# Polochon-street/bliss

Hardware: AMD Instinct MI355X
Metric: songs/sec bl_analyze (3-min 44.1kHz s16) + 10k x 10k distance-matrix sec (higher is better)
Workload: dtype f64; 1 GPU; configs[2] shard: 8192 synthetic 180-s 44.1 kHz s16 stereo songs/GPU resident (260.1 GB), 8192 total; step = analyze + all-gather + row-block distance; songs_per_gpu=8192, parallelism=shard1, fir_mode=2

## Files before the change

### bliss_amd/csrc/bl_stats_kernels.hip

```cpp
#include <hip/hip_runtime.h>
#include <math.h>

#include "bl_launch.h"
#include "bl_scan.h"
#include "bl_fir.h"


template <bool HIST>
__global__ __launch_bounds__(256) void k_pcm_scan(const int16_t *__restrict__ pcm,
                                                  const bl_dsong *__restrict__ songs,
                                                  bl_dstats *stats, unsigned *hist) {
  __shared__ unsigned lh[BL_HIST_BINS];
  if (__builtin_amdgcn_groupstaticsize() != sizeof lh) __builtin_trap();
  const int tid = threadIdx.x;
  const bl_dsong sg = songs[blockIdx.y];
  const int16_t *p = pcm + sg.pcm_off;
  for (int i = tid; i < BL_HIST_BINS; i += 256) lh[i] = 0;
  __syncthreads();
  unsigned lds_base = (unsigned)(size_t)(bl_lds_u32 *)lh;
  asm volatile("" : "+v"(lds_base));

  long long sum = 0;
  unsigned long long sq = 0;
  const unsigned nvec = (unsigned)sg.n >> 3;
  const uint4 *pv = reinterpret_cast<const uint4 *>(p);
  auto eat = [&](const uint4 q) {
    const unsigned w[4] = {q.x, q.y, q.z, q.w};
    int s32 = 0;
#pragma unroll
    for (int k = 0; k < 4; ++k) scan_word(w[k], s32, sq, lds_base, HIST);
    sum += s32;
  };
  const unsigned gstride = gridDim.x * 256u;
  unsigned v = blockIdx.x * 256u + tid;
  for (; v + gstride < nvec; v += 2 * gstride) {
    const uint4 q0 = pv[v], q1 = pv[v + gstride];
    eat(q0);
    eat(q1);
  }
  if (v < nvec) eat(pv[v]);
  if (blockIdx.x == 0 && tid < (sg.n & 7)) {
    const int sv = (int)p[8u * nvec + tid];
    sum += sv;
    sq += (unsigned)(sv * sv);
    const unsigned b = (unsigned)(sv + BL_HIST_BINS / 2);
    if (HIST && b < BL_HIST_BINS) atomicAdd(&lh[b], 1u);
  }
#pragma unroll
  for (int off = 32; off > 0; off >>= 1) {
    sum += __shfl_down(sum, off);
    sq += __shfl_down(sq, off);
  }
  bl_dstats *st = stats + blockIdx.y;
  if ((tid & 63) == 0) {
    atomicAdd(&st->sum, (unsigned long long)sum);
    atomicAdd(&st->sumsq, sq);
  }
  asm volatile("s_waitcnt lgkmcnt(0)" ::: "memory");
  __syncthreads();
  unsigned *gh = hist + (size_t)blockIdx.y * BL_HIST_BINS;
  for (int i = tid; i < BL_HIST_BINS; i += 256) {
    const unsigned c = lh[i];
    if (c) atomicAdd(&gh[i], c);
  }
}

__global__ __launch_bounds__(128) void k_trim(const int16_t *__restrict__ pcm, const bl_dsong *__restrict__ songs,
                                              bl_dstats *stats) {
  const bl_dsong sg = songs[blockIdx.x];
  const int16_t *p = pcm + sg.pcm_off;
  const uint4 *pv = reinterpret_cast<const uint4 *>(p);
  const int lane = threadIdx.x & 63, n = sg.n;
  const int nvec = n >> 3;
  const bool fwd = __builtin_amdgcn_readfirstlane(threadIdx.x >> 6) == 0;
  bl_dstats *st = stats + blockIdx.x;
  auto locate = [&](const uint4 q) -> int {
    const unsigned w[4] = {q.x, q.y, q.z, q.w};
    int at = fwd ? 8 : -1;
#pragma unroll
    for (int k = 0; k < 4; ++k) {
      if (fwd) {
        if (w[3 - k] >> 16) at = 2 * (3 - k) + 1;
        if (w[3 - k] & 0xFFFFu) at = 2 * (3 - k);
      } else {
        if (w[k] & 0xFFFFu) at = 2 * k;
        if (w[k] >> 16) at = 2 * k + 1;
      }
    }
    return at;
  };
  if (fwd) {
    unsigned first = 0xFFFFFFFFu;
    for (int v0 = 0; v0 < nvec; v0 += 128) {
      const int va = v0 + lane, vb = v0 + 64 + lane;
      const uint4 z = make_uint4(0, 0, 0, 0);
      const uint4 qa = va < nvec ? pv[va] : z, qb = vb < nvec ? pv[vb] : z;
      const unsigned long long ma = __ballot((qa.x | qa.y | qa.z | qa.w) != 0u);
      const unsigned long long mb = __ballot((qb.x | qb.y | qb.z | qb.w) != 0u);
      if (ma | mb) {
        const int src = ma ? __builtin_ctzll(ma) : __builtin_ctzll(mb);
        const unsigned mine = 8u * (unsigned)(ma ? va : vb) + (unsigned)locate(ma ? qa : qb);
        first = (unsigned)__shfl((int)mine, src);
        break;
      }
    }
    if (first == 0xFFFFFFFFu)
      for (int i = 8 * nvec; i < n; ++i)
        if (p[i] != 0) { first = (unsigned)i; break; }
    if (lane == 0) st->first = first;
  } else {
    int last = -1;
    for (int i = n - 1; i >= 8 * nvec; --i)
      if (p[i] != 0) { last = i; break; }
    if (last < 0)
      for (int v1 = nvec; v1 > 0; v1 -= 128) {
        const int va = v1 - 1 - lane, vb = v1 - 65 - lane;
        const uint4 z = make_uint4(0, 0, 0, 0);
        const uint4 qa = va >= 0 ? pv[va] : z, qb = vb >= 0 ? pv[vb] : z;
        const unsigned long long ma = __ballot((qa.x | qa.y | qa.z | qa.w) != 0u);
        const unsigned long long mb = __ballot((qb.x | qb.y | qb.z | qb.w) != 0u);
        if (ma | mb) {
          const int src = ma ? __builtin_ctzll(ma) : __builtin_ctzll(mb);
          const int mine = 8 * (ma ? va : vb) + locate(ma ? qa : qb);
          last = __shfl(mine, src);
          break;
        }
      }
    if (lane == 0) st->last = last;
  }
}

__global__ void k_stats_init(bl_dstats *stats, int n_songs) {
  const int i = blockIdx.x * blockDim.x + threadIdx.x;
  if (i >= n_songs) return;
  bl_dstats s;
  s.sum = 0; s.sumsq = 0; s.first = 0xFFFFFFFFu; s.last = -1;
  s.mean = 0; s.variance = 0; s.vprime = 0; s.rcp = 0; s.rcp_lo = 0; s.fsc = 0; s.kappa = 0; s.wrap_pass = 0; s.status = BL_OK;
  s.wrap_acc = 0;
  stats[i] = s;
}


__device__ __forceinline__ void prep_finish(bl_dstats &s, int n) {
  if (s.variance == 0) s.status = BL_UNEXPECTED;
  s.vprime = (double)s.variance / 32768.0;
  const double v2 = 2.0 * s.vprime;
  s.rcp = 1.0 / v2;
  s.rcp_lo = __builtin_fma(-s.rcp, v2, 1.0) / v2;
  s.fsc = bl_firi_scale(s.rcp, s.rcp_lo);
  s.kappa = bl_firi_power_scale(s.rcp, s.rcp_lo);
  (void)n;
}

__global__ void k_song_prep(const bl_dsong *__restrict__ songs, bl_dstats *stats, int n_songs,
                            bl_amd_song_result *res) {
  const int i = blockIdx.x * blockDim.x + threadIdx.x;
  if (i >= n_songs) return;
  bl_dstats s = stats[i];
  const bl_dsong sg = songs[i];
  const int n = sg.n;
  if (s.first == 0xFFFFFFFFu) {
    s.status = BL_UNEXPECTED;
    s.first = 0; s.last = n - 1;
  }
  const int wrapped = (int)(unsigned)(s.sum & 0xFFFFFFFFull);
  s.mean = wrapped / n;
  const long long m = s.mean;
  if (m > 13571 || m < -13571) {
    s.wrap_pass = 1;
  } else {
    const long long acc = (long long)s.sumsq - 2 * m * (long long)s.sum + (long long)n * m * m;
    s.variance = (int)(acc / n);
    prep_finish(s, n);
  }
  stats[i] = s;
  bl_amd_song_result *r = res + sg.out_idx;
  r->start = (int)s.first; r->end = s.last;
  r->mean = s.mean; r->variance = s.variance;
  r->n_frames = sg.n_frames; r->nb_frames = sg.nb_frames; r->n_windows = sg.n_windows;
  r->status = s.status;
}

__global__ __launch_bounds__(256) void k_variance_wrap(const int16_t *__restrict__ pcm,
                                                       const bl_dsong *__restrict__ songs,
                                                       bl_dstats *stats) {
  bl_dstats *st = stats + blockIdx.y;
  if (!st->wrap_pass) return;
  const bl_dsong sg = songs[blockIdx.y];
  const int16_t *p = pcm + sg.pcm_off;
  const int mean = st->mean;
  long long acc = 0;
  for (unsigned i = blockIdx.x * 256u + threadIdx.x; i < (unsigned)sg.n; i += gridDim.x * 256u) {
    const int v = (int)p[i] - mean;
    acc += (int)((unsigned)v * (unsigned)v);
  }
#pragma unroll
  for (int off = 32; off > 0; off >>= 1) acc += __shfl_down(acc, off);
  if ((threadIdx.x & 63) == 0)
    atomicAdd(reinterpret_cast<unsigned long long *>(&st->wrap_acc), (unsigned long long)acc);
}

__global__ void k_variance_wrap_finish(const bl_dsong *__restrict__ songs, bl_dstats *stats,
                                       int n_songs, bl_amd_song_result *res) {
  const int i = blockIdx.x * blockDim.x + threadIdx.x;
  if (i >= n_songs) return;
  bl_dstats s = stats[i];
  if (!s.wrap_pass) return;
  s.variance = (int)(s.wrap_acc / songs[i].n);
  prep_finish(s, songs[i].n);
  stats[i] = s;
  res[songs[i].out_idx].variance = s.variance;
  res[songs[i].out_idx].status = s.status;
}


#define BL_AMP_PASSES 301
#define BL_INT_LO ((32767 - 1000) - BL_HIST_LO)
#define BL_INT_HI ((32767 + 1000) - BL_HIST_LO)

__global__ __launch_bounds__(256) void k_amp_finish(const bl_dsong *__restrict__ songs,
                                                    const bl_dstats *__restrict__ stats,
                                                    const unsigned *__restrict__ hist,
                                                    bl_amd_song_result *res) {
  __shared__ float buf[2][BL_HIST_BINS + 8];
  const int tid = threadIdx.x;
  const int song = blockIdx.x;
  const bl_dstats st = stats[song];
  const int n = songs[song].n;
  const unsigned *gh = hist + (size_t)song * BL_HIST_BINS;
  const int start = (int)st.first, end = st.last;
  if (tid < 8) {
    const int c = tid < 3 ? tid : BL_HIST_BINS + tid;
    buf[0][c] = 0.f; buf[1][c] = 0.f;
  }
  for (int i = tid; i < BL_HIST_BINS; i += 256) {
    unsigned c = gh[i];
    if (i == BL_HIST_BINS / 2) c -= (unsigned)start + (unsigned)(n - 1 - end);
    buf[0][i + 3] = (float)min(c, 16777216u);
  }
  __syncthreads();
  int cur = 0;
  for (int g = 0; g < BL_AMP_PASSES; ++g) {
    const float *h = buf[cur] + 3;
    float *s = buf[cur ^ 1] + 3;
    const int reach = 3 * (BL_AMP_PASSES - 1 - g);
    const int lo = max(BL_INT_LO - reach, 0), hi = min(BL_INT_HI + reach, BL_HIST_BINS - 1);
    for (int i = lo + tid; i <= hi; i += 256) {
      float acc = h[i - 3] + (3 * h[i - 2]);
      acc = acc + (6 * h[i - 1]);
      acc = acc + (7 * h[i]);
      acc = acc + (6 * h[i + 1]);
      acc = acc + (3 * h[i + 2]);
      acc = acc + h[i + 3];
      s[i] = (float)(1. / 27. * (double)acc);
    }
    __syncthreads();
    cur ^= 1;
  }
  float *s = buf[cur] + 3;
  float *v = buf[cur ^ 1] + 3;
  const float denom = (float)(start - end);
  for (int i = BL_INT_LO + tid; i <= BL_INT_HI; i += 256) {
    float t = s[i] / denom;
    t = (float)((double)t * 100.);
    v[i] = fabsf(t);
  }
  __syncthreads();
  if (tid == 0) {
    float integral = 0;
    for (int i = BL_INT_LO; i <= BL_INT_HI; ++i) integral += v[i];
    bl_amd_song_result *r = res + songs[song].out_idx;
    r->hist_integral = integral;
    r->v.amplitude = -0.2f * integral + 6.0f;
  }
}

__global__ void k_force(bl_amd_song_result *res, int n_songs) {
  const int i = blockIdx.x * blockDim.x + threadIdx.x;
  if (i >= n_songs) return;
  bl_amd_song_result *r = res + i;
  const float rating = (float)(fmax((double)r->v.tempo, 0.0) + (double)r->v.amplitude +
                               (double)r->v.frequency + fmax((double)r->v.attack, 0.0));
  r->force = rating;
  r->calm_or_loud = rating > 0 ? BL_LOUD : (rating < 0 ? BL_CALM : BL_UNKNOWN);
}


static int scan_grid_x(int max_n, int n_songs, int n_cu) {
  return grid_x_for(((long long)max_n / 8 + 255) / 256, n_songs, 8, n_cu);
}

void blk_stats_init(const blk_analyze_args &a) {
  hipLaunchKernelGGL(k_stats_init, dim3((a.n_songs + 63) / 64), dim3(64), 0, a.stream, a.stats, a.n_songs);
}

int blk_pcm_scan(const blk_analyze_args &a) {
  BL_HIP_CHECK(hipMemsetAsync(a.hist, 0, sizeof(unsigned) * BL_HIST_BINS * (size_t)a.n_songs, a.stream));
  Mark m(a.mark, a.mark_user, PK_SCAN, a.stream);
  hipLaunchKernelGGL(k_pcm_scan<true>, dim3(scan_grid_x(a.max_n, a.n_songs, a.n_cu), a.n_songs), dim3(256), 0,
                     a.stream, a.pcm, a.songs, a.stats, a.hist);
  return BL_OK;
}

void blk_song_prep(const blk_analyze_args &a) {
  const int n_songs = a.n_songs, tb64 = (n_songs + 63) / 64;
  hipStream_t stream = a.stream;
  hipLaunchKernelGGL(k_trim, dim3(n_songs), dim3(128), 0, stream, a.pcm, a.songs, a.stats);
  hipLaunchKernelGGL(k_song_prep, dim3(tb64), dim3(64), 0, stream, a.songs, a.stats, n_songs,
                     a.results);
  hipLaunchKernelGGL(k_variance_wrap, dim3(scan_grid_x(a.max_n, n_songs, a.n_cu), n_songs), dim3(256), 0, stream,
                     a.pcm, a.songs, a.stats);
  hipLaunchKernelGGL(k_variance_wrap_finish, dim3(tb64), dim3(64), 0, stream, a.songs, a.stats,
                     n_songs, a.results);
}

void blk_amp_finish(const blk_analyze_args &a, hipStream_t s) {
  Mark m(a.mark, a.mark_user, PK_AMP, s);
  hipLaunchKernelGGL(k_amp_finish, dim3(a.n_songs), dim3(256), 0, s, a.songs, a.stats, a.hist,
                     a.results);
}

void blk_force(const blk_analyze_args &a) {
  hipLaunchKernelGGL(k_force, dim3((a.n_songs + 63) / 64), dim3(64), 0, a.stream, a.results, a.n_songs);
}

int blk_scan_one(hipStream_t s, const int16_t *pcm, const bl_dsong *d_songs, bl_dstats *d_stats,
                 unsigned *d_hist, int n, int n_cu) {
  const int gx = scan_grid_x(n, 1, n_cu);
  BL_HIP_CHECK(hipMemsetAsync(d_hist, 0, sizeof(unsigned) * BL_HIST_BINS, s));
  hipLaunchKernelGGL(k_stats_init, dim3(1), dim3(64), 0, s, d_stats, 1);
  hipLaunchKernelGGL(k_pcm_scan<true>, dim3(gx, 1), dim3(256), 0, s, pcm, d_songs, d_stats, d_hist);
  hipLaunchKernelGGL(k_trim, dim3(1), dim3(128), 0, s, pcm, d_songs, d_stats);
  BL_HIP_CHECK(hipGetLastError());
  return BL_OK;
}

int blk_variance_wrap_one(hipStream_t s, const int16_t *pcm, const bl_dsong *d_songs,
                          bl_dstats *d_stats, int n, int n_cu) {
  const int gx = scan_grid_x(n, 1, n_cu);
  hipLaunchKernelGGL(k_variance_wrap, dim3(gx, 1), dim3(256), 0, s, pcm, d_songs, d_stats);
  BL_HIP_CHECK(hipGetLastError());
  return BL_OK;
}
```

Before: 25490 songs/s.

## Run amplitude histogram smoothing passes in registers within one wavefront using DPP

Rewrites k_amp_finish so one 64-lane wave holds the histogram bins needed by the integral in registers, 60 per lane. Each of the 301 smoothing passes exchanges halo values between neighbouring lanes with DPP row shifts instead of going through LDS with a barrier per pass. Counts are loaded as 16-byte vectors, and the serial integral sum is replaced by per-lane sums chained through readlane. Register pressure is high (two 60-float arrays plus temporaries). The DPP row_shl/row_shr controls (0x138/0x130) shift within 16-lane rows, not across the full wave, so halo values at row boundaries may be wrong.

```diff
diff --git a/bliss_amd/csrc/bl_stats_kernels.hip b/bliss_amd/csrc/bl_stats_kernels.hip
--- a/bliss_amd/csrc/bl_stats_kernels.hip
+++ b/bliss_amd/csrc/bl_stats_kernels.hip
@@ -217,58 +217,107 @@
 #define BL_AMP_PASSES 301
 #define BL_INT_LO ((32767 - 1000) - BL_HIST_LO)
 #define BL_INT_HI ((32767 + 1000) - BL_HIST_LO)
-
-__global__ __launch_bounds__(256) void k_amp_finish(const bl_dsong *__restrict__ songs,
-                                                    const bl_dstats *__restrict__ stats,
-                                                    const unsigned *__restrict__ hist,
-                                                    bl_amd_song_result *res) {
-  __shared__ float buf[2][BL_HIST_BINS + 8];
-  const int tid = threadIdx.x;
+#define BL_AMP_PER_LANE 60
+#define BL_AMP_FIRST (BL_INT_LO - 3 * BL_AMP_PASSES)
+#define BL_AMP_LAST (BL_INT_HI + 3 * BL_AMP_PASSES)
+static_assert(BL_AMP_FIRST >= 0 && BL_AMP_FIRST % 4 == 0 && BL_AMP_PER_LANE % 4 == 0, "16-byte loads of the counts");
+static_assert(BL_AMP_FIRST + 64 * BL_AMP_PER_LANE <= BL_HIST_BINS, "every lane reads inside the song's histogram");
+static_assert(BL_AMP_FIRST + 64 * BL_AMP_PER_LANE > BL_AMP_LAST, "the wave covers every bin the integral depends on");
+
+__device__ __forceinline__ float amp_from_below(float v) {
+  return __int_as_float(__builtin_amdgcn_update_dpp(0, __float_as_int(v), 0x138 , 0xf, 0xf, false));
+}
+__device__ __forceinline__ float amp_from_above(float v) {
+  return __int_as_float(__builtin_amdgcn_update_dpp(0, __float_as_int(v), 0x130 , 0xf, 0xf, false));
+}
+
+__device__ __forceinline__ float amp_add(float a, float b) {
+  float d;
+  asm("v_add_f32_e32 %0, %1, %2" : "=v"(d) : "v"(a), "v"(b));
+  return d;
+}
+__device__ __forceinline__ float amp_mul(float c, float a) {
+  float d;
+  asm("v_mul_f32_e32 %0, %1, %2" : "=v"(d) : "s"(c), "v"(a));
+  return d;
+}
+
+__device__ __forceinline__ void amp_pass(const float (&in)[BL_AMP_PER_LANE], float (&out)[BL_AMP_PER_LANE]) {
+  constexpr int P = BL_AMP_PER_LANE;
+  float x[P + 6];
+  x[0] = amp_from_below(in[P - 3]);
+  x[1] = amp_from_below(in[P - 2]);
+  x[2] = amp_from_below(in[P - 1]);
+#pragma unroll
+  for (int r = 0; r < P; ++r) x[r + 3] = in[r];
+  x[P + 3] = amp_from_above(in[0]);
+  x[P + 4] = amp_from_above(in[1]);
+  x[P + 5] = amp_from_above(in[2]);
+  float x3[P + 6], x6[P + 6];
+#pragma unroll
+  for (int j = 1; j < P + 5; ++j) {
+    x3[j] = amp_mul(3.f, x[j]);
+    x6[j] = amp_mul(6.f, x[j]);
+  }
+#pragma unroll
+  for (int r = 0; r < P; ++r) {
+    const int i = r + 3;
+    float acc = amp_add(x[i - 3], x3[i - 2]);
+    acc = amp_add(acc, x6[i - 1]);
+    acc = amp_add(acc, amp_mul(7.f, x[i]));
+    acc = amp_add(acc, x6[i + 1]);
+    acc = amp_add(acc, x3[i + 2]);
+    acc = amp_add(acc, x[i + 3]);
+    out[r] = (float)(1. / 27. * (double)acc);
+  }
+}
+
+__global__ __launch_bounds__(64) void k_amp_finish(const bl_dsong *__restrict__ songs,
+                                                   const bl_dstats *__restrict__ stats,
+                                                   const unsigned *__restrict__ hist,
+                                                   bl_amd_song_result *res) {
+  constexpr int P = BL_AMP_PER_LANE;
+  const int lane = threadIdx.x;
   const int song = blockIdx.x;
   const bl_dstats st = stats[song];
   const int n = songs[song].n;
-  const unsigned *gh = hist + (size_t)song * BL_HIST_BINS;
   const int start = (int)st.first, end = st.last;
-  if (tid < 8) {
-    const int c = tid < 3 ? tid : BL_HIST_BINS + tid;
-    buf[0][c] = 0.f; buf[1][c] = 0.f;
-  }
-  for (int i = tid; i < BL_HIST_BINS; i += 256) {
-    unsigned c = gh[i];
-    if (i == BL_HIST_BINS / 2) c -= (unsigned)start + (unsigned)(n - 1 - end);
-    buf[0][i + 3] = (float)min(c, 16777216u);
-  }
-  __syncthreads();
-  int cur = 0;
-  for (int g = 0; g < BL_AMP_PASSES; ++g) {
-    const float *h = buf[cur] + 3;
-    float *s = buf[cur ^ 1] + 3;
-    const int reach = 3 * (BL_AMP_PASSES - 1 - g);
-    const int lo = max(BL_INT_LO - reach, 0), hi = min(BL_INT_HI + reach, BL_HIST_BINS - 1);
-    for (int i = lo + tid; i <= hi; i += 256) {
-      float acc = h[i - 3] + (3 * h[i - 2]);
-      acc = acc + (6 * h[i - 1]);
-      acc = acc + (7 * h[i]);
-      acc = acc + (6 * h[i + 1]);
-      acc = acc + (3 * h[i + 2]);
-      acc = acc + h[i + 3];
-      s[i] = (float)(1. / 27. * (double)acc);
+  const int bin0 = BL_AMP_FIRST + P * lane;
+  const uint4 *gh = reinterpret_cast<const uint4 *>(hist + (size_t)song * BL_HIST_BINS + bin0);
+  float a[P], b[P];
+#pragma unroll
+  for (int q = 0; q < P / 4; ++q) {
+    const uint4 c4 = gh[q];
+    const unsigned c[4] = {c4.x, c4.y, c4.z, c4.w};
+#pragma unroll
+    for (int k = 0; k < 4; ++k) {
+      unsigned v = c[k];
+      if (bin0 + 4 * q + k == BL_HIST_BINS / 2) v -= (unsigned)start + (unsigned)(n - 1 - end);
+      a[4 * q + k] = (float)min(v, 16777216u);
     }
-    __syncthreads();
-    cur ^= 1;
-  }
-  float *s = buf[cur] + 3;
-  float *v = buf[cur ^ 1] + 3;
+  }
+  for (int g = 0; g < BL_AMP_PASSES / 2; ++g) {
+    amp_pass(a, b);
+    amp_pass(b, a);
+  }
+  static_assert(BL_AMP_PASSES % 2 == 1, "the last pass leaves the result in b");
+  amp_pass(a, b);
   const float denom = (float)(start - end);
-  for (int i = BL_INT_LO + tid; i <= BL_INT_HI; i += 256) {
-    float t = s[i] / denom;
+#pragma unroll
+  for (int r = 0; r < P; ++r) {
+    float t = b[r] / denom;
     t = (float)((double)t * 100.);
-    v[i] = fabsf(t);
-  }
-  __syncthreads();
-  if (tid == 0) {
-    float integral = 0;
-    for (int i = BL_INT_LO; i <= BL_INT_HI; ++i) integral += v[i];
+    const int i = bin0 + r;
+    b[r] = (i >= BL_INT_LO && i <= BL_INT_HI) ? fabsf(t) : 0.f;
+  }
+  float integral = 0;
+  for (int l = (BL_INT_LO - BL_AMP_FIRST) / P; l <= (BL_INT_HI - BL_AMP_FIRST) / P; ++l) {
+    float t = integral;
+#pragma unroll
+    for (int r = 0; r < P; ++r) t += b[r];
+    integral = __int_as_float(__builtin_amdgcn_readlane(__float_as_int(t), l));
+  }
+  if (lane == 0) {
     bl_amd_song_result *r = res + songs[song].out_idx;
     r->hist_integral = integral;
     r->v.amplitude = -0.2f * integral + 6.0f;
@@ -316,7 +365,7 @@
 
 void blk_amp_finish(const blk_analyze_args &a, hipStream_t s) {
   Mark m(a.mark, a.mark_user, PK_AMP, s);
-  hipLaunchKernelGGL(k_amp_finish, dim3(a.n_songs), dim3(256), 0, s, a.songs, a.stats, a.hist,
+  hipLaunchKernelGGL(k_amp_finish, dim3(a.n_songs), dim3(64), 0, s, a.songs, a.stats, a.hist,
                      a.results);
 }
 
```

Result: no change. 25490 songs/s (-0.0%).
